# ViktorLiang/GW-Depth

Hardware: AMD Instinct MI355X
Metric: images/sec (train fwd+bwd) 480x640 bs=8/GPU (higher is better)
Workload: dtype bf16; 1 GPU; GW-Depth full model (res50 + DETR 6+6 + 4-scale ReferTransformer + decoder) fwd+17 losses+bwd+clip+AdamW, 480x640, bs=8/GPU, dropout 0.1; global_batch=8, parallelism=dp1, launch=hipgraph, graph_segments=1, grad_buckets=8

## Files before the change

gw_depth_amd/csrc/refattn.hip:

```cpp
#include "common.h"

namespace {

struct QOp {
    const void *p;
    long ws, ts, hs;
};
struct QOpW {
    void *p;
    long ws, ts, hs;
};

template <typename T, int HD>
__device__ __forceinline__ void load_row(float (&v)[HD], const T *p) {
    if constexpr (sizeof(T) == 2) {
#pragma unroll
        for (int c = 0; c < HD; c += 8) {
            const bf16x8 x = *(const bf16x8 *)(p + c);
#pragma unroll
            for (int j = 0; j < 8; ++j) v[c + j] = (float)x[j];
        }
    } else {
#pragma unroll
        for (int c = 0; c < HD; c += 4) {
            const float4 x = *(const float4 *)(p + c);
            v[c] = x.x, v[c + 1] = x.y, v[c + 2] = x.z, v[c + 3] = x.w;
        }
    }
}

template <typename T, int HD>
__global__ void ref_scores_fwd_kernel(QOp q, const T *__restrict__ refk, T *__restrict__ ra, int B, int nwin, int R, int H, float scale) {
    const long total = (long)B * nwin * 49 * H;
    const int C = H * HD, Tn = nwin * 49;
    for (long i = (long)blockIdx.x * blockDim.x + threadIdx.x; i < total; i += (long)gridDim.x * blockDim.x) {
        const int h = (int)(i % H);
        const long bt = i / H;
        const int t = (int)(bt % Tn), b = (int)(bt / Tn);
        float qv[HD];
        load_row<T, HD>(qv, (const T *)q.p + ((long)b * nwin + t / 49) * q.ws + (long)(t % 49) * q.ts + (long)h * q.hs);
        const T *kp = refk + (long)b * R * C + h * HD;
        T *dst = ra + bt * R * H + h;
        for (int r = 0; r < R; ++r) {
            float kv[HD];
            load_row<T, HD>(kv, kp + (long)r * C);
            float acc = 0.f;
#pragma unroll
            for (int d = 0; d < HD; ++d) acc += qv[d] * kv[d];
            dst[(long)r * H] = from_f32<T>(acc * scale);
        }
    }
}

template <typename T, int HD>
__global__ void ref_scores_dq_kernel(const T *__restrict__ refk, const T *__restrict__ g, QOpW dq, int B, int nwin, int R, int H, float scale) {
    const long total = (long)B * nwin * 49 * H;
    const int C = H * HD, Tn = nwin * 49;
    for (long i = (long)blockIdx.x * blockDim.x + threadIdx.x; i < total; i += (long)gridDim.x * blockDim.x) {
        const int h = (int)(i % H);
        const long bt = i / H;
        const int t = (int)(bt % Tn), b = (int)(bt / Tn);
        const T *gp = g + bt * R * H + h;
        const T *kp = refk + (long)b * R * C + h * HD;
        float acc[HD];
#pragma unroll
        for (int d = 0; d < HD; ++d) acc[d] = 0.f;
        for (int r = 0; r < R; ++r) {
            float kv[HD];
            load_row<T, HD>(kv, kp + (long)r * C);
            const float gv = to_f32(gp[(long)r * H]);
#pragma unroll
            for (int d = 0; d < HD; ++d) acc[d] += gv * kv[d];
        }
        T *dst = (T *)dq.p + ((long)b * nwin + t / 49) * dq.ws + (long)(t % 49) * dq.ts + (long)h * dq.hs;
#pragma unroll
        for (int d = 0; d < HD; ++d) dst[d] = from_f32<T>(acc[d] * scale);
    }
}

template <typename T, int HD>
__global__ void token_reduce_kernel(const T *__restrict__ a, QOp x, float *__restrict__ out, int B, int nwin, int R, int H, float scale) {
    const int lane = threadIdx.x & 63;
    const long wave = ((long)blockIdx.x * blockDim.x + threadIdx.x) >> 6, total = (long)B * R * H;
    if (wave >= total) return;
    const int h = (int)(wave % H), r = (int)((wave / H) % R), b = (int)(wave / ((long)H * R));
    const int Tn = nwin * 49;
    const T *ap = a + ((long)b * Tn * R + r) * H + h;
    float acc[HD];
#pragma unroll
    for (int d = 0; d < HD; ++d) acc[d] = 0.f;
    for (int t = lane; t < Tn; t += 64) {
        float xv[HD];
        load_row<T, HD>(xv, (const T *)x.p + ((long)b * nwin + t / 49) * x.ws + (long)(t % 49) * x.ts + (long)h * x.hs);
        const float av = to_f32(ap[(long)t * R * H]);
#pragma unroll
        for (int d = 0; d < HD; ++d) acc[d] += av * xv[d];
    }
    float *dst = out + ((long)b * R + r) * H * HD + h * HD;
#pragma unroll
    for (int d = 0; d < HD; ++d) {
        const float s = wave_sum(acc[d]);
        if (lane == (d & 63)) dst[d] = s * scale;
    }
}

template <typename T>
__global__ void ref_mix_fwd_kernel(const T *__restrict__ ra, const T *__restrict__ refv, T *__restrict__ qnew, T *__restrict__ att_out,
                                   int R, int H, int hd, int Tn) {
    extern __shared__ float sm[];
    const long bt = blockIdx.x;
    const int C = H * hd, RH = R * H;
    const T *src = ra + bt * RH;
    for (int e = threadIdx.x; e < RH; e += blockDim.x) sm[e] = to_f32(src[e]);
    __syncthreads();
    {
        float *red = sm + RH;
        const int parts = blockDim.x / H, hh = threadIdx.x % H, pp = threadIdx.x / H;
        float m = -INFINITY;
        if (pp < parts)
            for (int r = pp; r < R; r += parts) m = fmaxf(m, sm[r * H + hh]);
        if (pp < parts) red[pp * H + hh] = m;
        __syncthreads();
        for (int q = 0; q < parts; ++q) m = fmaxf(m, red[q * H + hh]);
        __syncthreads();
        float l = 0.f;
        if (pp < parts)
            for (int r = pp; r < R; r += parts) {
                const float p = __expf(sm[r * H + hh] - m);
                sm[r * H + hh] = p;
                l += p;
            }
        if (pp < parts) red[pp * H + hh] = l;
        __syncthreads();
        l = 0.f;
        for (int q = 0; q < parts; ++q) l += red[q * H + hh];
        const float inv = 1.0f / l;
        if (pp < parts)
            for (int r = pp; r < R; r += parts) sm[r * H + hh] *= inv;
    }
    __syncthreads();
    if (att_out)
        for (int e = threadIdx.x; e < RH; e += blockDim.x) att_out[bt * RH + e] = from_f32<T>(sm[e]);
    const T *vb = refv + (bt / Tn) * R * C;
    for (int e = threadIdx.x; e < C; e += blockDim.x) {
        const int h = e / hd;
        float acc = 0.f;
        for (int r = 0; r < R; ++r) acc += sm[r * H + h] * to_f32(vb[(long)r * C + e]);
        qnew[bt * C + e] = from_f32<T>(acc);
    }
}

template <typename T>
__global__ void ref_mix_bwd_kernel(const T *__restrict__ att, const T *__restrict__ refv, const T *__restrict__ g, T *__restrict__ dra,
                                   int R, int H, int hd, int Tn) {
    extern __shared__ float sm[];
    const long bt = blockIdx.x;
    const int C = H * hd, RH = R * H;
    const int GP = hd + 1;
    float *gs = sm, *da = sm + H * GP, *dot = da + RH;
    for (int e = threadIdx.x; e < C; e += blockDim.x) gs[(e / hd) * GP + e % hd] = to_f32(g[bt * C + e]);
    __syncthreads();
    const T *vb = refv + (bt / Tn) * R * C;
    constexpr int VE = 16 / (int)sizeof(T);
    const bool vec = (hd % VE) == 0 && ((uintptr_t)vb % 16) == 0;
    for (int e = threadIdx.x; e < RH; e += blockDim.x) {
        const int r = e / H, h = e % H;
        const T *vp = vb + (long)r * C + h * hd;
        float acc = 0.f;
        if (vec) {
            for (int d = 0; d < hd; d += VE) {
                const uint4 raw = *(const uint4 *)(vp + d);
                const T *pv = (const T *)&raw;
#pragma unroll
                for (int k = 0; k < VE; ++k) acc += gs[h * GP + d + k] * to_f32(pv[k]);
            }
        } else {
            for (int d = 0; d < hd; ++d) acc += gs[h * GP + d] * to_f32(vp[d]);
        }
        da[e] = acc;
    }
    __syncthreads();
    float *part = dot + H;
    const int parts = blockDim.x / H, hh = threadIdx.x % H, pp = threadIdx.x / H;
    float av[4];
    float s = 0.f;
    int n = 0;
    if (pp < parts)
        for (int r = pp; r < R; r += parts, ++n) {
            const float a = to_f32(att[bt * RH + r * H + hh]);
            if (n < 4) av[n] = a;
            s += a * da[r * H + hh];
        }
    if (pp < parts) part[pp * H + hh] = s;
    __syncthreads();
    if (threadIdx.x < H) {
        float t = 0.f;
        for (int q = 0; q < parts; ++q) t += part[q * H + threadIdx.x];
        dot[threadIdx.x] = t;
    }
    __syncthreads();
    n = 0;
    if (pp < parts)
        for (int r = pp; r < R; r += parts, ++n) {
            const float a = n < 4 ? av[n] : to_f32(att[bt * RH + r * H + hh]);
            dra[bt * RH + r * H + hh] = from_f32<T>(a * (da[r * H + hh] - dot[hh]));
        }
}

bool shape_ok(int B, int nwin, int R, int H, int hd) { return B > 0 && nwin > 0 && R > 0 && R <= 128 && H > 0 && H <= 64 && hd > 0 && hd <= 64; }
int blocks_for(long n, int per, int cap) {
    long b = (n + per - 1) / per;
    return (int)(b > cap ? cap : (b < 1 ? 1 : b));
}

}

#define HD_SWITCH(hd, CALL)            \
    switch (hd) {                      \
        case 8: { CALL(8) } break;     \
        case 16: { CALL(16) } break;   \
        case 32: { CALL(32) } break;   \
        case 64: { CALL(64) } break;   \
        default: return -4;            \
    }

bool q_aligned(const gwd_strided *q, int32_t dtype) {
    const int a = dtype == GWD_BF16 ? 8 : 4;
    return (uintptr_t)q->p % 16 == 0 && q->ws % a == 0 && q->ts % a == 0 && q->hs % a == 0;
}

extern "C" int gwd_ref_scores_forward(const gwd_strided *q, const void *ref_k, void *ra, int32_t B, int32_t nwin, int32_t R, int32_t H,
                                      int32_t hd, float scale, int32_t dtype, void *stream) {
    if (!q || !q->p || !ref_k || !ra || !shape_ok(B, nwin, R, H, hd)) return -1;
    if (!q_aligned(q, dtype) || (uintptr_t)ref_k % 16) return -5;
    const QOp qo{q->p, q->ws, q->ts, q->hs};
    const int grid = blocks_for((long)B * nwin * 49 * H, 64, 16384);
    hipStream_t s = (hipStream_t)stream;
    if (dtype == GWD_BF16) {
#define CALL(HD_) ref_scores_fwd_kernel<__bf16, HD_><<<grid, 64, 0, s>>>(qo, (const __bf16 *)ref_k, (__bf16 *)ra, B, nwin, R, H, scale);
        HD_SWITCH(hd, CALL)
#undef CALL
    } else if (dtype == GWD_F32) {
#define CALL(HD_) ref_scores_fwd_kernel<float, HD_><<<grid, 64, 0, s>>>(qo, (const float *)ref_k, (float *)ra, B, nwin, R, H, scale);
        HD_SWITCH(hd, CALL)
#undef CALL
    } else return -2;
    GWD_CHECK_LAUNCH();
    return 0;
}

extern "C" int gwd_ref_scores_backward(const gwd_strided *q, const void *ref_k, const void *g, const gwd_strided *dq, float *d_ref_k,
                                       int32_t B, int32_t nwin, int32_t R, int32_t H, int32_t hd, float scale, int32_t dtype,
                                       void *stream) {
    if (!q || !q->p || !dq || !dq->p || !ref_k || !g || !d_ref_k || !shape_ok(B, nwin, R, H, hd)) return -1;
    if (!q_aligned(q, dtype) || (uintptr_t)ref_k % 16) return -5;
    const QOp qo{q->p, q->ws, q->ts, q->hs};
    const QOpW dqo{dq->p, dq->ws, dq->ts, dq->hs};
    const int grid = blocks_for((long)B * nwin * 49 * H, 64, 16384);
    const unsigned rgrid = (unsigned)(((long)B * R * H + 3) / 4);
    hipStream_t s = (hipStream_t)stream;
    if (dtype == GWD_BF16) {
#define CALL(HD_)                                                                                                             \
    ref_scores_dq_kernel<__bf16, HD_><<<grid, 64, 0, s>>>((const __bf16 *)ref_k, (const __bf16 *)g, dqo, B, nwin, R, H, scale);    \
    token_reduce_kernel<__bf16, HD_><<<rgrid, 256, 0, s>>>((const __bf16 *)g, qo, d_ref_k, B, nwin, R, H, scale);
        HD_SWITCH(hd, CALL)
#undef CALL
    } else if (dtype == GWD_F32) {
#define CALL(HD_)                                                                                                             \
    ref_scores_dq_kernel<float, HD_><<<grid, 64, 0, s>>>((const float *)ref_k, (const float *)g, dqo, B, nwin, R, H, scale);       \
    token_reduce_kernel<float, HD_><<<rgrid, 256, 0, s>>>((const float *)g, qo, d_ref_k, B, nwin, R, H, scale);
        HD_SWITCH(hd, CALL)
#undef CALL
    } else return -2;
    GWD_CHECK_LAUNCH();
    return 0;
}

extern "C" int gwd_ref_mix_forward(const void *ra, const void *ref_v, void *q_new, void *att, int32_t B, int32_t T, int32_t R, int32_t H,
                                   int32_t hd, int32_t dtype, void *stream) {
    if (!ra || !ref_v || !q_new || T <= 0 || !shape_ok(B, 1, R, H, hd)) return -1;
    const unsigned grid = (unsigned)((long)B * T);
    hipStream_t s = (hipStream_t)stream;
    const size_t lds = ((size_t)R * H + (size_t)(256 / H) * H) * sizeof(float);
    if (dtype == GWD_BF16) ref_mix_fwd_kernel<__bf16><<<grid, 256, lds, s>>>((const __bf16 *)ra, (const __bf16 *)ref_v, (__bf16 *)q_new, (__bf16 *)att, R, H, hd, T);
    else if (dtype == GWD_F32) ref_mix_fwd_kernel<float><<<grid, 256, lds, s>>>((const float *)ra, (const float *)ref_v, (float *)q_new, (float *)att, R, H, hd, T);
    else return -2;
    GWD_CHECK_LAUNCH();
    return 0;
}

extern "C" int gwd_ref_mix_backward(const void *att, const void *ref_v, const void *g, void *d_ra, float *d_ref_v, int32_t B, int32_t T,
                                    int32_t R, int32_t H, int32_t hd, int32_t dtype, void *stream) {
    if (!att || !ref_v || !g || !d_ra || !d_ref_v || T <= 0 || T % 49 || !shape_ok(B, 1, R, H, hd)) return -1;
    if ((uintptr_t)g % 16) return -5;
    hipStream_t s = (hipStream_t)stream;
    const size_t lds = ((size_t)H * (hd + 1) + (size_t)R * H + H + (size_t)(256 / H) * H) * sizeof(float);
    const unsigned rgrid = (unsigned)(((long)B * R * H + 3) / 4);
    const long C = (long)H * hd;
    const QOp go{g, 49 * C, C, hd};
    if (dtype == GWD_BF16) {
        ref_mix_bwd_kernel<__bf16><<<(unsigned)((long)B * T), 256, lds, s>>>((const __bf16 *)att, (const __bf16 *)ref_v, (const __bf16 *)g, (__bf16 *)d_ra, R, H, hd, T);
#define CALL(HD_) token_reduce_kernel<__bf16, HD_><<<rgrid, 256, 0, s>>>((const __bf16 *)att, go, d_ref_v, B, T / 49, R, H, 1.0f);
        HD_SWITCH(hd, CALL)
#undef CALL
    } else if (dtype == GWD_F32) {
        ref_mix_bwd_kernel<float><<<(unsigned)((long)B * T), 256, lds, s>>>((const float *)att, (const float *)ref_v, (const float *)g, (float *)d_ra, R, H, hd, T);
#define CALL(HD_) token_reduce_kernel<float, HD_><<<rgrid, 256, 0, s>>>((const float *)att, go, d_ref_v, B, T / 49, R, H, 1.0f);
        HD_SWITCH(hd, CALL)
#undef CALL
    } else return -2;
    GWD_CHECK_LAUNCH();
    return 0;
}
```

Before: 266.4 images/s.

## Restructure reference-attention score and token-reduce kernels with slicing and LDS staging

Replaces the per-thread loop over all reference rows in the scores forward with a 2D grid that slices references in groups of 8 and batches the key loads. The dQ backward now splits each head dimension into 8-element pieces with vectorized loads and stores. The token reduction uses a new 1024-thread kernel that stages attention weights in LDS, has many threads split the token axis, and sums the partial results in shared memory. The goal is better parallelism and memory coalescing for the reference-attention kernels, at the cost of more code paths, fallback branches and a large LDS footprint.

After: 268.4 images/s, median of 6. No clear change (+0.8%).

```diff
diff --git a/gw_depth_amd/csrc/refattn.hip b/gw_depth_amd/csrc/refattn.hip
--- a/gw_depth_amd/csrc/refattn.hip
+++ b/gw_depth_amd/csrc/refattn.hip
@@ -29,28 +29,127 @@
     }
 }
 
-template <typename T, int HD>
-__global__ void ref_scores_fwd_kernel(QOp q, const T *__restrict__ refk, T *__restrict__ ra, int B, int nwin, int R, int H, float scale) {
-    const long total = (long)B * nwin * 49 * H;
-    const int C = H * HD, Tn = nwin * 49;
-    for (long i = (long)blockIdx.x * blockDim.x + threadIdx.x; i < total; i += (long)gridDim.x * blockDim.x) {
-        const int h = (int)(i % H);
-        const long bt = i / H;
-        const int t = (int)(bt % Tn), b = (int)(bt / Tn);
+template <typename T, int N> struct RawRow;
+template <int N> struct RawRow<__bf16, N> {
+    bf16x8 v[N / 8];
+    __device__ __forceinline__ void load(const __bf16 *p) {
+#pragma unroll
+        for (int c = 0; c < N / 8; ++c) v[c] = *(const bf16x8 *)(p + c * 8);
+    }
+    __device__ __forceinline__ __bf16 raw(int d) const { return v[d / 8][d % 8]; }
+    __device__ __forceinline__ float at(int d) const { return (float)raw(d); }
+};
+template <int N> struct RawRow<float, N> {
+    f32x4 v[N / 4];
+    __device__ __forceinline__ void load(const float *p) {
+#pragma unroll
+        for (int c = 0; c < N / 4; ++c) v[c] = *(const f32x4 *)(p + c * 4);
+    }
+    __device__ __forceinline__ float raw(int d) const { return v[d / 4][d % 4]; }
+    __device__ __forceinline__ float at(int d) const { return raw(d); }
+};
+
+__device__ __forceinline__ void store_row8(__bf16 *p, const float (&v)[8]) {
+    bf16x8 o;
+#pragma unroll
+    for (int j = 0; j < 8; ++j) o[j] = (__bf16)v[j];
+    *(bf16x8 *)p = o;
+}
+__device__ __forceinline__ void store_row8(float *p, const float (&v)[8]) {
+    *(f32x4 *)p = f32x4{v[0], v[1], v[2], v[3]};
+    *(f32x4 *)(p + 4) = f32x4{v[4], v[5], v[6], v[7]};
+}
+
+__device__ __forceinline__ void divmod(long n, int d, long &q, int &r) {
+    if (n < (1L << 32)) {
+        const unsigned un = (unsigned)n, uq = un / (unsigned)d;
+        q = uq, r = (int)(un - uq * (unsigned)d);
+    } else {
+        q = n / d, r = (int)(n % d);
+    }
+}
+
+constexpr int kRefSlice = 8;
+
+template <typename T, int HD>
+__global__ void __launch_bounds__(256) ref_scores_fwd_sliced_kernel(QOp q, const T *__restrict__ refk, T *__restrict__ ra, int B, int nwin, int R, int H, float scale) {
+    constexpr int ROWS = 256 / (HD * (int)sizeof(T)), NB = ROWS < 1 ? 1 : (ROWS > kRefSlice ? kRefSlice : ROWS);
+    const long per_slice = (long)B * nwin * 49 * H;
+    const int C = H * HD, Tn = nwin * 49, r0 = (int)blockIdx.y * kRefSlice;
+    for (long i = (long)blockIdx.x * blockDim.x + threadIdx.x; i < per_slice; i += (long)gridDim.x * blockDim.x) {
+        long bt, bl;
+        int h, t;
+        divmod(i, H, bt, h);
+        divmod(bt, Tn, bl, t);
+        const int b = (int)bl;
         float qv[HD];
         load_row<T, HD>(qv, (const T *)q.p + ((long)b * nwin + t / 49) * q.ws + (long)(t % 49) * q.ts + (long)h * q.hs);
         const T *kp = refk + (long)b * R * C + h * HD;
         T *dst = ra + bt * R * H + h;
-        for (int r = 0; r < R; ++r) {
-            float kv[HD];
-            load_row<T, HD>(kv, kp + (long)r * C);
-            float acc = 0.f;
-#pragma unroll
-            for (int d = 0; d < HD; ++d) acc += qv[d] * kv[d];
-            dst[(long)r * H] = from_f32<T>(acc * scale);
-        }
-    }
-}
+#pragma unroll
+        for (int j0 = 0; j0 < kRefSlice; j0 += NB) {
+            RawRow<T, HD> kv[NB];
+#pragma unroll
+            for (int j = 0; j < NB; ++j) {
+                const int r = r0 + j0 + j;
+                kv[j].load(kp + (long)(r < R ? r : R - 1) * C);
+            }
+#pragma unroll
+            for (int j = 0; j < NB; ++j) {
+                const int r = r0 + j0 + j;
+                float acc = 0.f;
+#pragma unroll
+                for (int d = 0; d < HD; ++d) acc += qv[d] * kv[j].at(d);
+                if (r < R) dst[(long)r * H] = from_f32<T>(acc * scale);
+            }
+        }
+    }
+}
+
+template <typename T, int HD>
+__global__ void __launch_bounds__(256) ref_scores_dq_piece_kernel(const T *__restrict__ refk, const T *__restrict__ g, QOpW dq, int B, int nwin, int R, int H, float scale) {
+    constexpr int P = HD / 8;
+    const long total = (long)B * nwin * 49 * H * P;
+    const int C = H * HD, Tn = nwin * 49;
+    for (long i = (long)blockIdx.x * blockDim.x + threadIdx.x; i < total; i += (long)gridDim.x * blockDim.x) {
+        const int p = (int)(i % P);
+        long bt, bl;
+        int h, t;
+        divmod(i / P, H, bt, h);
+        divmod(bt, Tn, bl, t);
+        const int b = (int)bl;
+        const T *gp = g + bt * R * H + h;
+        const T *kp = refk + (long)b * R * C + h * HD + p * 8;
+        float acc[8];
+#pragma unroll
+        for (int d = 0; d < 8; ++d) acc[d] = 0.f;
+        int r = 0;
+        for (; r + kRefSlice <= R; r += kRefSlice) {
+            RawRow<T, 8> kv[kRefSlice];
+            float gv[kRefSlice];
+#pragma unroll
+            for (int j = 0; j < kRefSlice; ++j) {
+                kv[j].load(kp + (long)(r + j) * C);
+                gv[j] = to_f32(gp[(long)(r + j) * H]);
+            }
+#pragma unroll
+            for (int j = 0; j < kRefSlice; ++j)
+#pragma unroll
+                for (int d = 0; d < 8; ++d) acc[d] += gv[j] * kv[j].at(d);
+        }
+        for (; r < R; ++r) {
+            RawRow<T, 8> kv;
+            kv.load(kp + (long)r * C);
+            const float gv = to_f32(gp[(long)r * H]);
+#pragma unroll
+            for (int d = 0; d < 8; ++d) acc[d] += gv * kv.at(d);
+        }
+#pragma unroll
+        for (int d = 0; d < 8; ++d) acc[d] *= scale;
+        store_row8((T *)dq.p + ((long)b * nwin + t / 49) * dq.ws + (long)(t % 49) * dq.ts + (long)h * dq.hs + p * 8, acc);
+    }
+}
+
 
 template <typename T, int HD>
 __global__ void ref_scores_dq_kernel(const T *__restrict__ refk, const T *__restrict__ g, QOpW dq, int B, int nwin, int R, int H, float scale) {
@@ -75,6 +174,87 @@
         T *dst = (T *)dq.p + ((long)b * nwin + t / 49) * dq.ws + (long)(t % 49) * dq.ts + (long)h * dq.hs;
 #pragma unroll
         for (int d = 0; d < HD; ++d) dst[d] = from_f32<T>(acc[d] * scale);
+    }
+}
+
+constexpr int kRedGroup = 2, kRedThreads = 1024, kRedUnroll = 8, kRedStageBytes = 60 * 1024;
+
+template <typename T, int HD, int G>
+__global__ void __launch_bounds__(kRedThreads) token_reduce_rows_kernel(const T *__restrict__ a, QOp x, float *__restrict__ out, int B, int nwin, int R, int H, int chunk, float scale) {
+    extern __shared__ __attribute__((aligned(16))) unsigned char lds[];
+    typedef T AV __attribute__((ext_vector_type(G)));
+    T *as = (T *)lds;
+    float *part = (float *)lds;
+    const int NC = H * (HD / 8), row = NC * 8, splits = (int)blockDim.x / NC;
+    const int b = (int)blockIdx.x % B, r0 = ((int)blockIdx.x / B) * G;
+    const int Tn = nwin * 49;
+    const int c = (int)threadIdx.x % NC, s = (int)threadIdx.x / NC, h = c / (HD / 8);
+    const T *ab = a + (long)b * Tn * R * H;
+    const T *xb = (const T *)x.p + (long)b * nwin * x.ws + c * 8;
+    const int xts = (int)x.ts, xwadj = (int)(x.ws - 49 * x.ts);
+    constexpr int VE = 16 / (int)sizeof(T);
+    const bool vec = r0 + G <= R && H % VE == 0 && (uintptr_t)a % 16 == 0;
+    float acc[G][8];
+#pragma unroll
+    for (int g = 0; g < G; ++g)
+#pragma unroll
+        for (int j = 0; j < 8; ++j) acc[g][j] = 0.f;
+    for (int t0 = 0; t0 < Tn; t0 += chunk) {
+        const int n = Tn - t0 < chunk ? Tn - t0 : chunk;
+        if (t0) __syncthreads();
+        if (vec) {
+            const int ppt = G * H / VE;
+            for (int i = (int)threadIdx.x; i < n * ppt; i += (int)blockDim.x) {
+                const int tl = i / ppt, e0 = (i % ppt) * VE, g = e0 / H, h0 = e0 % H;
+                RawRow<T, VE> v;
+                v.load(ab + ((long)(t0 + tl) * R + r0) * H + e0);
+#pragma unroll
+                for (int k = 0; k < VE; ++k) as[((long)tl * H + h0 + k) * G + g] = v.raw(k);
+            }
+        } else {
+            for (int i = (int)threadIdx.x; i < n * G * H; i += (int)blockDim.x) {
+                const int tl = i / (G * H), e = i % (G * H), g = e / H, hh = e % H;
+                as[((long)tl * H + hh) * G + g] = ab[((long)(t0 + tl) * R + (r0 + g < R ? r0 + g : R - 1)) * H + hh];
+            }
+        }
+        __syncthreads();
+        if (s < splits)
+            for (int tl = s; tl < n; tl += kRedUnroll * splits) {
+                RawRow<T, 8> xv[kRedUnroll];
+#pragma unroll
+                for (int u = 0; u < kRedUnroll; ++u) {
+                    const int t = t0 + (tl + u * splits < n ? tl + u * splits : tl);
+                    int off = t * xts;
+                    if (xwadj) off += (t / 49) * xwadj;
+                    xv[u].load(xb + off);
+                }
+#pragma unroll
+                for (int u = 0; u < kRedUnroll; ++u)
+                    if (tl + u * splits < n) {
+                        const AV av = *(const AV *)(as + ((long)(tl + u * splits) * H + h) * G);
+#pragma unroll
+                        for (int g = 0; g < G; ++g)
+#pragma unroll
+                            for (int j = 0; j < 8; ++j) acc[g][j] += to_f32(av[g]) * xv[u].at(j);
+                    }
+            }
+    }
+    __syncthreads();
+    if (s < splits) {
+#pragma unroll
+        for (int g = 0; g < G; ++g) {
+            float *dst = part + ((long)(s * G + g) * NC + c) * 8;
+            *(f32x4 *)dst = f32x4{acc[g][0], acc[g][1], acc[g][2], acc[g][3]};
+            *(f32x4 *)(dst + 4) = f32x4{acc[g][4], acc[g][5], acc[g][6], acc[g][7]};
+        }
+    }
+    __syncthreads();
+    for (int o = (int)threadIdx.x; o < G * row; o += (int)blockDim.x) {
+        const int g = o / row, e = o % row;
+        if (r0 + g >= R) break;
+        float sum = 0.f;
+        for (int k = 0; k < splits; ++k) sum += part[(long)(k * G + g) * row + e];
+        out[((long)b * R + r0 + g) * row + e] = sum * scale;
     }
 }
 
@@ -213,6 +393,41 @@
     return (int)(b > cap ? cap : (b < 1 ? 1 : b));
 }
 
+template <typename T, int HD>
+void launch_token_reduce(const T *a, const QOp &x, float *out, int B, int nwin, int R, int H, float scale, hipStream_t s) {
+    const auto fits = [](long v) { return v < (1L << 30) && v > -(1L << 30); };
+    if (x.hs == HD && fits(nwin * x.ws) && fits(nwin * 49 * x.ts)) {
+        const int NC = H * (HD / 8), splits = kRedThreads / NC, Tn = nwin * 49;
+        const int fit = kRedStageBytes / (kRedGroup * H * (int)sizeof(T)), chunk = Tn < fit ? Tn : fit;
+        const size_t stage = (size_t)chunk * kRedGroup * H * sizeof(T);
+        const size_t sums = (size_t)splits * kRedGroup * NC * 8 * sizeof(float);
+        const unsigned grid = (unsigned)((long)B * ((R + kRedGroup - 1) / kRedGroup));
+        token_reduce_rows_kernel<T, HD, kRedGroup><<<grid, kRedThreads, stage > sums ? stage : sums, s>>>(a, x, out, B, nwin, R, H, chunk, scale);
+    } else {
+        const unsigned grid = (unsigned)(((long)B * R * H + 3) / 4);
+        token_reduce_kernel<T, HD><<<grid, 256, 0, s>>>(a, x, out, B, nwin, R, H, scale);
+    }
+}
+
+template <typename T, int HD>
+void launch_scores_fwd(const QOp &q, const void *ref_k, void *ra, int B, int nwin, int R, int H, float scale, hipStream_t s) {
+    const dim3 grid(blocks_for((long)B * nwin * 49 * H, 256, 16384), (R + kRefSlice - 1) / kRefSlice);
+    ref_scores_fwd_sliced_kernel<T, HD><<<grid, 256, 0, s>>>(q, (const T *)ref_k, (T *)ra, B, nwin, R, H, scale);
+}
+
+template <typename T, int HD>
+void launch_scores_bwd(const QOp &q, const void *ref_k, const void *g, const QOpW &dq, float *d_ref_k, int B, int nwin, int R, int H,
+                       float scale, hipStream_t s) {
+    constexpr int A = 16 / (int)sizeof(T);
+    if ((uintptr_t)dq.p % 16 == 0 && dq.ws % A == 0 && dq.ts % A == 0 && dq.hs % A == 0) {
+        const long n = (long)B * nwin * 49 * H * (HD / 8);
+        ref_scores_dq_piece_kernel<T, HD><<<blocks_for(n, 256, 16384), 256, 0, s>>>((const T *)ref_k, (const T *)g, dq, B, nwin, R, H, scale);
+    } else {
+        ref_scores_dq_kernel<T, HD><<<blocks_for((long)B * nwin * 49 * H, 64, 16384), 64, 0, s>>>((const T *)ref_k, (const T *)g, dq, B, nwin, R, H, scale);
+    }
+    launch_token_reduce<T, HD>((const T *)g, q, d_ref_k, B, nwin, R, H, scale, s);
+}
+
 }
 
 #define HD_SWITCH(hd, CALL)            \
@@ -234,14 +449,13 @@
     if (!q || !q->p || !ref_k || !ra || !shape_ok(B, nwin, R, H, hd)) return -1;
     if (!q_aligned(q, dtype) || (uintptr_t)ref_k % 16) return -5;
     const QOp qo{q->p, q->ws, q->ts, q->hs};
-    const int grid = blocks_for((long)B * nwin * 49 * H, 64, 16384);
     hipStream_t s = (hipStream_t)stream;
     if (dtype == GWD_BF16) {
-#define CALL(HD_) ref_scores_fwd_kernel<__bf16, HD_><<<grid, 64, 0, s>>>(qo, (const __bf16 *)ref_k, (__bf16 *)ra, B, nwin, R, H, scale);
+#define CALL(HD_) launch_scores_fwd<__bf16, HD_>(qo, ref_k, ra, B, nwin, R, H, scale, s);
         HD_SWITCH(hd, CALL)
 #undef CALL
     } else if (dtype == GWD_F32) {
-#define CALL(HD_) ref_scores_fwd_kernel<float, HD_><<<grid, 64, 0, s>>>(qo, (const float *)ref_k, (float *)ra, B, nwin, R, H, scale);
+#define CALL(HD_) launch_scores_fwd<float, HD_>(qo, ref_k, ra, B, nwin, R, H, scale, s);
         HD_SWITCH(hd, CALL)
 #undef CALL
     } else return -2;
@@ -256,19 +470,13 @@
     if (!q_aligned(q, dtype) || (uintptr_t)ref_k % 16) return -5;
     const QOp qo{q->p, q->ws, q->ts, q->hs};
     const QOpW dqo{dq->p, dq->ws, dq->ts, dq->hs};
-    const int grid = blocks_for((long)B * nwin * 49 * H, 64, 16384);
-    const unsigned rgrid = (unsigned)(((long)B * R * H + 3) / 4);
     hipStream_t s = (hipStream_t)stream;
     if (dtype == GWD_BF16) {
-#define CALL(HD_)                                                                                                             \
-    ref_scores_dq_kernel<__bf16, HD_><<<grid, 64, 0, s>>>((const __bf16 *)ref_k, (const __bf16 *)g, dqo, B, nwin, R, H, scale);    \
-    token_reduce_kernel<__bf16, HD_><<<rgrid, 256, 0, s>>>((const __bf16 *)g, qo, d_ref_k, B, nwin, R, H, scale);
+#define CALL(HD_) launch_scores_bwd<__bf16, HD_>(qo, ref_k, g, dqo, d_ref_k, B, nwin, R, H, scale, s);
         HD_SWITCH(hd, CALL)
 #undef CALL
     } else if (dtype == GWD_F32) {
-#define CALL(HD_)                                                                                                             \
-    ref_scores_dq_kernel<float, HD_><<<grid, 64, 0, s>>>((const float *)ref_k, (const float *)g, dqo, B, nwin, R, H, scale);       \
-    token_reduce_kernel<float, HD_><<<rgrid, 256, 0, s>>>((const float *)g, qo, d_ref_k, B, nwin, R, H, scale);
+#define CALL(HD_) launch_scores_bwd<float, HD_>(qo, ref_k, g, dqo, d_ref_k, B, nwin, R, H, scale, s);
         HD_SWITCH(hd, CALL)
 #undef CALL
     } else return -2;
@@ -295,17 +503,16 @@
     if ((uintptr_t)g % 16) return -5;
     hipStream_t s = (hipStream_t)stream;
     const size_t lds = ((size_t)H * (hd + 1) + (size_t)R * H + H + (size_t)(256 / H) * H) * sizeof(float);
-    const unsigned rgrid = (unsigned)(((long)B * R * H + 3) / 4);
     const long C = (long)H * hd;
     const QOp go{g, 49 * C, C, hd};
     if (dtype == GWD_BF16) {
         ref_mix_bwd_kernel<__bf16><<<(unsigned)((long)B * T), 256, lds, s>>>((const __bf16 *)att, (const __bf16 *)ref_v, (const __bf16 *)g, (__bf16 *)d_ra, R, H, hd, T);
-#define CALL(HD_) token_reduce_kernel<__bf16, HD_><<<rgrid, 256, 0, s>>>((const __bf16 *)att, go, d_ref_v, B, T / 49, R, H, 1.0f);
+#define CALL(HD_) launch_token_reduce<__bf16, HD_>((const __bf16 *)att, go, d_ref_v, B, T / 49, R, H, 1.0f, s);
         HD_SWITCH(hd, CALL)
 #undef CALL
     } else if (dtype == GWD_F32) {
         ref_mix_bwd_kernel<float><<<(unsigned)((long)B * T), 256, lds, s>>>((const float *)att, (const float *)ref_v, (const float *)g, (float *)d_ra, R, H, hd, T);
-#define CALL(HD_) token_reduce_kernel<float, HD_><<<rgrid, 256, 0, s>>>((const float *)att, go, d_ref_v, B, T / 49, R, H, 1.0f);
+#define CALL(HD_) launch_token_reduce<float, HD_>((const float *)att, go, d_ref_v, B, T / 49, R, H, 1.0f, s);
         HD_SWITCH(hd, CALL)
 #undef CALL
     } else return -2;
```
